# oriolfornes/ExplaiNN

Measured on AMD Instinct MI355X. Metric: sequences/sec (fwd+bwd), 200bp one-hot, 300 units, batch 1024, higher is better.
Workload: dtype f32

## Files before the change

explainn_amd/csrc/api.hip:

```cpp
#include <stdarg.h>
#include <stdio.h>
#include <string.h>

#include <cstdlib>
#include <cstring>

#include "common.h"

static thread_local char g_err[512] = "";

void explainn_set_error(const char* fmt, ...) {
    va_list ap;
    va_start(ap, fmt);
    vsnprintf(g_err, sizeof(g_err), fmt, ap);
    va_end(ap);
}

extern "C" const char* explainn_last_error(void) { return g_err; }

namespace {
struct Carver {
    int64_t off = 0;
    char* base = nullptr;
    template <typename T>
// ... 22 lines not shown
    cv.take(&c->Wsg, (int64_t)conv_tiles_padded(c->U, c->k) * 32);
    const int64_t Upad = (int64_t)32 * conv_tiles_padded(c->U, c->k);
    cv.take(&c->ext, Upad * n * Bs + 64);
    cv.take(&c->idx, Upad * n * Bs + 64);
    cv.take(&c->qs0, U * NS);
    cv.take(&c->qS1p, U * c->QCH * NS);
    cv.take(&c->qS2p, U * c->QCH * NS * NS);
    cv.take(&c->qbar, U * NS);
    cv.take(&c->VC, U * FC_H * NS);
    cv.take(&c->A2, U * FC_H * NS);
    cv.take(&c->A2f, c->NQ <= FC_BF_MAXN ? 0 : U * FC_MT * fc_nk4q(c->NQ) * 256);
    cv.take(&c->A2h, c->NQ <= FC_BF_MAXN ? U * FC_MT * fc_ks32(c->NQ) * 3 * 256 : 0);
    cv.take(&c->sh2, U * FC_H);
    cv.take(&c->sig2, U * FC_H);
    cv.take(&c->z, U * Bs);
    cv.take(&c->zhat, U * Bs);
    cv.take(&c->o, U * Bs);
    cv.take(&c->sig3, U);
    c->ZBLK = fc_fwd_blocks((int)Bs, c->NQ);
    cv.take(&c->z12p, U * c->ZBLK * 2);
    cv.take(&c->bits, U * Bs + 4);
    cv.take(&c->dz, U * Bs + 4);
    cv.take(&c->EQp, U * c->ACH * FC_H * NS);
    cv.take(&c->Sep, U * c->ACH * FC_H);
    cv.take(&c->EQs, U * FC_H * NS);
    cv.take(&c->Ttf, U * fc_nw16(c->NQ) * 3 * 4 * 256);
    cv.take(&c->Mff, U * fc_nw16(c->NQ) * 4 * fc_nw16(c->NQ) * 64);
    cv.take(&c->k0p, U * NS);
    cv.take(&c->dy, U4 * n * Bs);
    cv.take(&c->S12p, U * fc_ng(c->NQ) * (Bs / 16) * 2);
    cv.take(&c->Dspp, U * (Bs / 4) * K4);
    cv.take(&c->dlogits, (int64_t)c->maxB * c->T);
    cv.take(&c->flags, 64);
    cv.take(&c->dlT, (int64_t)c->T * Bs);
    cv.take(&c->gWp, c->T > HEAD_GEMM_MIN_T ? (int64_t)head_gw_chunks(c->maxB) * c->T * (c->U + 1) : 0);
    cv.take(&c->lossp, 256);
    cv.take(&c->site_cnt, U4 * Bs);
    cv.take(&c->site_off, U4 * Bs);
    cv.off = (cv.off + 255) & ~int64_t(255);
}

int check_batch(const explainn_ctx* c, int B) {
    if (!c) { explainn_set_error("null context"); return EXPLAINN_E_ARG; }
    if (B < 1 || B > c->maxB) {
        explainn_set_error("batch %d outside [1, max_batch=%d]", B, c->maxB);
        return EXPLAINN_E_ARG;
    }
    return EXPLAINN_OK;
}

#define TRY(call)                    \
    do {                             \
        int rc_ = (call);            \
        if (rc_ != EXPLAINN_OK) return rc_; \
    } while (0)

const char* const kStageNames[ST_COUNT] = {
    "pack_tables", "moments", "prep1_stats", "conv_pool", "qmom", "prep2", "fc_fwd", "head_fwd",
    "loss", "head_bwd", "passA", "mid", "passB", "conv_bwd", "fin_bwd"};
#define STAGE(id, call)                                                                 \
    do {                                                                                \
        if (c->timing) HIP_TRY(hipEventRecord(c->ev0[id], s));                          \
        TRY(call);                                                                      \
        if (c->timing) { HIP_TRY(hipEventRecord(c->ev1[id], s)); c->timed |= 1u << (id); } \
    } while (0)

// ... 187 lines not shown
}

extern "C" int explainn_forward_train(explainn_ctx* c, const float* x, int B,
                                      const explainn_params* p, const uint8_t* keep_mask,
                                      float dropout_p, uint64_t seed, float* logits, void* stream) {
    TRY(check_batch(c, B));
    if (B == 1) {
        explainn_set_error("Expected more than 1 value per channel when training, got input size "
                           "[1, %d, 1]", FC_H * c->U);
        return EXPLAINN_E_BATCH1;
    }
    if (dropout_p < 0.f || dropout_p >= 1.f) {
        explainn_set_error("dropout_p must be in [0,1)");
        return EXPLAINN_E_ARG;
    }
    hipStream_t s = static_cast<hipStream_t>(stream);
    c->fwd_B = 0;
    c->eval_valid = false;
    c->dense_x = nullptr;
    if (c->dense) {
        if (!x) { explainn_set_error("dense input mode needs x"); return EXPLAINN_E_ARG; }
        c->staged_B = 0;
        STAGE(ST_PACK, launch_prep1_tables(c, p, s));
        STAGE(ST_MOMENTS, launch_dense_moments(c, x, B, s));
        STAGE(ST_PREP1, launch_prep1(c, p, B, true, s));
        STAGE(ST_CONV_POOL, launch_dense_conv_pool(c, x, p, B, s));
        c->dense_x = x;
    } else {
    if (x) STAGE(ST_PACK, launch_pack_tables(c, x, p, B, s));
    else {
        TRY(launch_pack(c, x, B, false, s));
        STAGE(ST_PACK, launch_prep1_tables(c, p, s));
    }
    STAGE(ST_MOMENTS, launch_moments(c, B, s));
    STAGE(ST_PREP1, launch_prep1(c, p, B, true, s));
    STAGE(ST_CONV_POOL, launch_conv_pool(c, p, B, true, s));
    }
    STAGE(ST_QMOM, launch_qmoments(c, B, s));
    STAGE(ST_PREP2, launch_prep2(c, p, B, true, s));
    STAGE(ST_FC_FWD, launch_fc_fwd(c, p, B, true, keep_mask, dropout_p, seed, s));
    STAGE(ST_HEAD_FWD, launch_head_fwd(c, p, B, true, logits, nullptr, s));
    c->fwd_B = B;
    return EXPLAINN_OK;
}

namespace {
int backward_fc(explainn_ctx* c, int B, const explainn_params* p, const explainn_grads* g,
                const pa_head_args* head, hipStream_t s) {
    STAGE(ST_PASSA, launch_passA(c, B, head, s));
    STAGE(ST_MID, launch_mid_bwd(c, p, g, B, s));
    return EXPLAINN_OK;
}

int backward_conv(explainn_ctx* c, int B, const explainn_params* p, const explainn_grads* g,
                  int freeze_top_n_filters, hipStream_t s) {
    STAGE(ST_PASSB, launch_passB(c, B, s));
    if (c->dense_x) STAGE(ST_CONV_BWD, launch_dense_conv_bwd(c, c->dense_x, B, s));
    else STAGE(ST_CONV_BWD, launch_conv_bwd(c, B, s));
    STAGE(ST_FIN, launch_fin_bwd(c, p, g, B, freeze_top_n_filters, s));
    return EXPLAINN_OK;
}

bool head_rides_in_passA(const explainn_ctx* c, int B) { return c->T <= PA_HEAD_MAX_T && B <= 512; }

pa_head_args head_in_passA(explainn_ctx* c, const explainn_params* p, const explainn_grads* g, int mode,
                           const float* dl, int kind, const float* logits, const float* y,
                           float* loss_out) {
    pa_head_args h = {mode, c->T, kind, dl, logits, y, loss_out, p->final_w, p->bn3_w, c->o, c->zhat,
                      c->sig3, c->dz, g->final_w, g->final_b, g->bn3_w, g->bn3_b, g->fc2_b};
// ... 166 lines not shown
```

explainn_amd/csrc/common.h:

```cpp
#pragma once
#include <hip/hip_runtime.h>
#include <stdint.h>

#include "../../include/explainn_hip.h"

#define FC_H 100
#define HEAD_RB 8
#define HEAD_GEMM_MIN_T 8
#define HEAD_GW_MAXCH 32
__host__ inline int head_gw_chunks(int B) { int c = (B + 127) / 128; return c < 1 ? 1 : (c > HEAD_GW_MAXCH ? HEAD_GW_MAXCH : c); }
#define POOLW 7
#define BN_EPS_D 1e-5
#define BN_MOM_D 0.1
#define WAVE 64
#define MAX_K 32
#define MAX_NQ 160

struct explainn_ctx {
    int U, k, L, T, maxB, device;
    int Lo, n;
    int U4, Uq;
    int NQ, NS;
    int Bs;
    int K4;
// ... 33 lines not shown
    float* A2f;
    float* A2h;
    float* sh2;
    float* sig2;
    float* z;
    float* zhat;
    float* o;
    float* sig3;
    double* z12p;
    int ZBLK;
    uint4* bits;
    float* dz;
    float* EQp;
    float* Sep;
    float* EQs;
    float* Ttf;
    float* Mff;
    float* k0p;
    float* dy;
    float* S12p;
    float* Dspp;
    int dsp_stride, dsp_count;
    float* dlogits;
    float* dlT;
    int loss_blocks, loss_n; float* loss_out;
    float* gWp;
    double* lossp;
    int staged_B;
    bool eval_valid;
    uint64_t eval_version;
    bool dense;
    const float* dense_x;
    int* flags;
    int* site_cnt;
    int* site_off;
};

enum explainn_stage {
    ST_PACK, ST_MOMENTS, ST_PREP1, ST_CONV_POOL, ST_QMOM, ST_PREP2, ST_FC_FWD, ST_HEAD_FWD, ST_LOSS,
    ST_HEAD_BWD, ST_PASSA, ST_MID, ST_PASSB, ST_CONV_BWD, ST_FIN, ST_COUNT
};

void explainn_set_error(const char* fmt, ...);
#define HIP_TRY(expr)                                                              \
    do {                                                                           \
        hipError_t e_ = (expr);                                                    \
        if (e_ != hipSuccess) {                                                    \
            explainn_set_error("%s failed: %s (%s:%d)", #expr, hipGetErrorString(e_), \
                               __FILE__, __LINE__);                                \
            (void)hipGetLastError();   \
            return EXPLAINN_E_HIP;                                                 \
        }                                                                          \
    } while (0)
#define LAUNCH_CHECK()  HIP_TRY(hipGetLastError())

int launch_pack(explainn_ctx* c, const float* x, int B, bool counts, hipStream_t s);
int launch_prep1(explainn_ctx* c, const explainn_params* p, int B, bool train, hipStream_t s);
int launch_moments(explainn_ctx* c, int B, hipStream_t s);
int launch_prep1_tables(explainn_ctx* c, const explainn_params* p, hipStream_t s);
int launch_conv_pool(explainn_ctx* c, const explainn_params* p, int B, bool want_idx, hipStream_t s);
int launch_pack_tables(explainn_ctx* c, const float* x, const explainn_params* p, int B, hipStream_t s);
int launch_pack_codes(explainn_ctx* c, const uint8_t* codes, int B, int rc, hipStream_t s);
int launch_conv_act(explainn_ctx* c, int B, float* acts, hipStream_t s);
int launch_filter_act_max(explainn_ctx* c, int B, const uint8_t* select, float* umax, hipStream_t s);
int launch_filter_sites(explainn_ctx* c, int B, const uint8_t* select, const float* thr, int cap,
                        int* site_total, int* pfm, uint8_t* hit, hipStream_t s);
int launch_qmoments(explainn_ctx* c, int B, hipStream_t s);
int launch_prep2(explainn_ctx* c, const explainn_params* p, int B, bool train, hipStream_t s);
int launch_fc_fwd(explainn_ctx* c, const explainn_params* p, int B, bool train,
                  const uint8_t* keep_mask, float drop_p, uint64_t seed, hipStream_t s);
int launch_head_fwd(explainn_ctx* c, const explainn_params* p, int B, bool train, float* logits,
                    float* outs, hipStream_t s);
int launch_loss_deferred(explainn_ctx* c, int kind, const float* logits, const float* y, int B, float* loss,
                         float* dlogits, hipStream_t s);
int launch_loss(explainn_ctx* c, int kind, const float* logits, const float* y, int B,
                float* loss, float* dlogits, hipStream_t s);
int launch_head_bwd(explainn_ctx* c, const explainn_params* p, const explainn_grads* g,
                    const float* dlogits, int B, hipStream_t s);
int launch_head_bwd_fused_loss(explainn_ctx* c, const explainn_params* p, const explainn_grads* g,
                               int kind, const float* logits, const float* y, float* loss_out, int B,
                               hipStream_t s);
#define PA_HEAD_MAX_T 4
struct pa_head_args {
    int mode, T, kind;
    const float *dl, *logits, *y;
    float* loss_out;
    const float *Wf, *g3, *o, *zhat, *sig3;
    float *dz, *gWf, *gbf, *gg3, *gb3, *gc2;
};
int launch_passA(explainn_ctx* c, int B, const pa_head_args* head, hipStream_t s);
int launch_mid_bwd(explainn_ctx* c, const explainn_params* p, const explainn_grads* g, int B,
                   hipStream_t s);
int launch_passB(explainn_ctx* c, int B, hipStream_t s);
// ... 54 lines not shown
    const float sgn = (u < U && gamma1[u] < 0.f) ? -1.f : 1.f;
    if (tid == 0) Wsg[((u >> 5) * 2 + ((u >> 2) & 1)) * 16 + 4 * ((u & 31) >> 3) + (u & 3)] = sgn < 0.f ? 0x80000000u : 0u;
    for (int kk = tid; kk < 16 * KS; kk += nthreads) {
        const int j = kk >> 2, a = kk & 3;
        const float wv = j < k ? sgn * wsh[a * k + j] : 0.f;
        const uint32_t hb = __float_as_uint(wv) & 0xffff0000u;
        const float r1 = wv - __uint_as_float(hb);
        const uint32_t mb = __float_as_uint(r1) & 0xffff0000u;
        const float r2 = r1 - __uint_as_float(mb);
        const int ks = kk >> 4, lane = 32 * ((kk >> 3) & 1) + (u & 31), e = kk & 7;
        uint16_t* dst = Wf + ((((size_t)(u >> 5) * KS + ks) * 3) * 64 + lane) * 8 + e;
        dst[0] = (uint16_t)(hb >> 16);
        dst[512] = (uint16_t)(mb >> 16);
        dst[1024] = (uint16_t)(__float_as_uint(r2) >> 16);
    }
}

#ifndef EXPLAINN_XCD_MAP
#define EXPLAINN_XCD_MAP 1
#endif
__device__ __forceinline__ bool unit_chunk_of_block(int U, int& u, int& chunk) {
#if EXPLAINN_XCD_MAP
    const int G = gridDim.x, L = blockIdx.y * G + blockIdx.x;
    const int slot = L >> 3;
    u = (slot / G) * 8 + (L & 7);
    chunk = slot - (slot / G) * G;
#else
    u = blockIdx.y; chunk = blockIdx.x;
#endif
    return u < U;
}
__host__ inline int units_grid(int U) { return (U + 7) & ~7; }

__device__ __forceinline__ float qval(float alpha, float ext, float shift) {
    return __expf(fmaf(alpha, ext, shift));
}

__device__ __forceinline__ float wave_sum(float v) {
#pragma unroll
    for (int off = 32; off > 0; off >>= 1) v += __shfl_xor(v, off, 64);
    return v;
}
__device__ __forceinline__ double wave_sum_d(double v) {
#pragma unroll
    for (int off = 32; off > 0; off >>= 1) v += __shfl_xor(v, off, 64);
    return v;
}

__host__ __device__ constexpr int chunk_count(int len) { return (len + 35) / 36; }
__host__ __device__ constexpr int chunk_len(int len) {
    return (((len + chunk_count(len) - 1) / chunk_count(len)) + 3) & ~3;
}
__host__ __device__ constexpr int ns_stride(int NQ) { return chunk_count(NQ) * chunk_len(NQ); }

static inline int nq_bucket(int n) {
    static const int b[] = {4, 8, 12, 16, 20, 24, 26, 28, 32, 40, 48, 56, 64, 72, 84, 96,
                            112, 128, 140, 160};
    for (unsigned i = 0; i < sizeof(b) / sizeof(b[0]); ++i)
        if (b[i] >= n) return b[i];
    return 0;
}
__host__ __device__ constexpr int nq_lower(int NQ) {
    constexpr int b[] = {0, 4, 8, 12, 16, 20, 24, 26, 28, 32, 40, 48, 56, 64, 72, 84, 96, 112, 128, 140, 160};
    int lo = 0;
    for (int i = 1; i < 21; ++i) if (b[i] == NQ) lo = b[i - 1];
    return lo;
// ... 33 lines not shown
```

explainn_amd/csrc/convpool.hip:

```cpp
#include <cstdlib>
#include <type_traits>

#include "common.h"

typedef __attribute__((ext_vector_type(8))) __bf16 cbf16x8;
typedef float cf32x16 __attribute__((ext_vector_type(16)));
typedef uint32_t cu32x4 __attribute__((ext_vector_type(4)));

template <int KS, int UT> struct cpm_state {
    cu32x4 Wr[UT][KS][3];
    cf32x16 acc[3][UT];
    float best[UT][16];
    uint32_t arg[UT][16];
    cu32x4 bop[3][KS];
    uint32_t xs[3], nx[2];
    uint32_t gw[4], mw[3];
    uint32_t smask[UT][16];
    uint32_t so, so4;
    uint32_t r1, r5;
};
struct cpm_args {
    const uint32_t* pk2; const uint32_t* nmask; float* ext; uint8_t* idx;
    int n, Bs, PW, NW, t0, b, kh; uint32_t tbase;
    uint32_t row1, row5;
// ... 155 lines not shown
                    cpm_update_sel<KS, UT, IDX, PI, RP>(S, (e - 1) / 16, (e - 1) % 16, gt[(e - 1) % 3]);
                    cpm_update_sel<KS, UT, IDX, PI, RP>(S, e / 16, e % 16, gt[e % 3]);
                }
            } else {
                constexpr int e = k - SC::E0 - SC::NE;
                cpm_store<KS, UT, IDX>(S, A, e / 16, e % 16);
            }
        });
        __builtin_amdgcn_sched_barrier(0);
    });
}

template <int KS, int UT, bool IDX>
__device__ __forceinline__ void cpm_window(cpm_state<KS, UT>& S, const cpm_args& A, int w) {
    cpm_position<KS, UT, IDX, 0>(S, A, w);
    cpm_position<KS, UT, IDX, 1>(S, A, w);
    cpm_position<KS, UT, IDX, 2>(S, A, w);
    cpm_position<KS, UT, IDX, 3>(S, A, w);
    cpm_position<KS, UT, IDX, 4>(S, A, w);
    cpm_position<KS, UT, IDX, 5>(S, A, w);
    cpm_position<KS, UT, IDX, 6>(S, A, w);
}

template <int KS, int UT>
__device__ __forceinline__ void cpm_load_fragments(cpm_state<KS, UT>& S, const cu32x4* wsrc) {
    cpm_static_for<0, UT * KS * 3>([&S, wsrc](auto ic) {
        constexpr int i = decltype(ic)::value;
        cu32x4& dst = S.Wr[i / (KS * 3)][(i / 3) % KS][i % 3];
        const cu32x4* src = wsrc + 64 * i;
        asm volatile("global_load_dwordx4 %0, %1, off" : "=a"(dst) : "v"(src));
    });
}

template <int KS, int UT, bool IDX>
__global__ __launch_bounds__(64, (UT == 1 && KS <= 5) ? 2 : 1) void conv_pool_mm_kernel(
    const uint32_t* __restrict__ pk2, const uint32_t* __restrict__ nmask,
    const cu32x4* __restrict__ Wf, const cu32x4* __restrict__ Wsg,
    float* __restrict__ ext, uint8_t* __restrict__ idx, int n, int Bs, int PW, int NW, int wper) {
    __shared__ __attribute__((aligned(1024))) cu32x4 oh[64];
    typedef __attribute__((address_space(3))) char lds_char;
    const int lane = threadIdx.x;
    STAMP(0);
    {
        const int c4 = lane & 15, nb = lane >> 4;
        uint32_t r[4] = {0u, 0u, 0u, 0u};
#pragma unroll
        for (int h = 0; h < 2; ++h) {
            const int cde = (c4 >> (2 * h)) & 3;
            const uint32_t one = ((nb >> h) & 1) ? 0u : 0x3F80u;
#pragma unroll
            for (int q = 0; q < 4; ++q)
                if (q == 2 * h + (cde >> 1)) r[q] = one << (16 * (cde & 1));
        }
        oh[lane] = cu32x4{r[0], r[1], r[2], r[3]};
    }
    cpm_state<KS, UT> S;
    cpm_args A;
    A.pk2 = pk2; A.nmask = nmask; A.ext = ext; A.idx = idx; A.n = n; A.Bs = Bs; A.PW = PW; A.NW = NW;
    A.t0 = blockIdx.y * UT; A.b = blockIdx.x * 32 + (lane & 31); A.kh = lane >> 5;
    A.tbase = (uint32_t)(size_t)(const lds_char*)oh;
    A.row1 = (uint32_t)(n * Bs); A.row5 = 5u * A.row1;
    {
        const size_t row0 = (size_t)32 * A.t0 * n * Bs;
        const int span = __builtin_amdgcn_readfirstlane(32 * UT * n * Bs);
        auto uniform = [](auto* q) {
            const unsigned long long v = reinterpret_cast<unsigned long long>(q);
            const unsigned lo = __builtin_amdgcn_readfirstlane((unsigned)v), hi = __builtin_amdgcn_readfirstlane((unsigned)(v >> 32));
            return reinterpret_cast<decltype(q)>(((unsigned long long)hi << 32) | lo);
        };
        A.rext = __builtin_amdgcn_make_buffer_rsrc(uniform(ext + row0), 0, 4 * span, 0x00020000);
        A.ridx = __builtin_amdgcn_make_buffer_rsrc(uniform(idx + row0), 0, span, 0x00020000);
    }
    const int wbeg = blockIdx.z * wper, wend = min(n, wbeg + wper);
    if (wbeg >= wend) return;
    cpm_load_fragments(S, Wf + (size_t)A.t0 * KS * 3 * 64 + lane);
    cpm_fetch(S, A, wbeg);
    {
        const cu32x4* ssrc = Wsg + ((size_t)A.t0 * 2 + A.kh) * 4;
#pragma unroll
        for (int t = 0; t < UT; ++t)
#pragma unroll
            for (int q = 0; q < 4; ++q) {
                const cu32x4 v = ssrc[t * 8 + q];
#pragma unroll
                for (int i = 0; i < 4; ++i) S.smask[t][4 * q + i] = v[i];
            }
    }
    asm volatile("s_waitcnt vmcnt(0)" ::: "memory");
    __syncthreads();
    STAMP(1);
    cpm_window_words(S, A, wbeg);
    cpm_static_for<0, KS>([&](auto kc) { cpm_operand<KS, UT, 0, decltype(kc)::value, 0>(S, A); });
    STAMP(2);
#pragma unroll 1
    for (int w = wbeg; w < wend; ++w) {
        const bool first = w == wbeg;
        S.so = first ? CPM_OOB : cpm_store_origin(A, w - 1);
        S.so4 = first ? CPM_OOB : 4u * S.so;
        S.r1 = first ? 0u : A.row1; S.r5 = first ? 0u : A.row5;
        cpm_window<KS, UT, IDX>(S, A, w);
        if (first) STAMP(3);
    }
    STAMP(4);
    __builtin_amdgcn_sched_barrier(0);
    asm volatile("s_nop 15\n\ts_nop 15\n\ts_nop 15" ::: "memory");
    __builtin_amdgcn_sched_barrier(0);
// ... 2 lines not shown
#pragma unroll
        for (int r = 0; r < 16; ++r) cpm_update<KS, UT, IDX, POOLW - 1, 2>(S, t, r);
    S.so = cpm_store_origin(A, wend - 1);
    S.so4 = 4u * S.so;
    S.r1 = A.row1; S.r5 = A.row5;
#pragma unroll
    for (int t = 0; t < UT; ++t)
#pragma unroll
        for (int r = 0; r < 16; ++r) cpm_store<KS, UT, IDX>(S, A, t, r);
    STAMP(5);
}

static int conv_pool_mm_ut(const explainn_ctx* c) {
    if (const char* e = getenv("EXPLAINN_CPM_UT")) { const int v = atoi(e); if (v == 1 || (v == 2 && conv_ksteps(c->k) <= 5)) return v; }
    return conv_ut(c->k);
}

static int conv_pool_mm_parts(const explainn_ctx* c, int B, int ut) {
    if (const char* e = getenv("EXPLAINN_CPM_PARTS")) { const int v = atoi(e); if (v >= 1) return min(v, c->n); }
    const int groups = ut == 1 ? (c->U + 31) / 32 : conv_tiles_padded(c->U, c->k) / ut, sb = (B + 31) / 32;
    const int cols = groups * sb, slots = (ut == 1 && conv_ksteps(c->k) <= 5) ? 2048 : 1024;
    int best = 1;
    long best_cost = -1;
    for (int p = 1; p <= c->n; ++p) {
        const int wper = (c->n + p - 1) / p, np = (c->n + wper - 1) / wper;
        if (np != p) continue;
        const long rounds = ((long)cols * np + slots - 1) / slots;
        const long cost = rounds * (wper + 1);
        if (best_cost < 0 || cost < best_cost) { best_cost = cost; best = p; }
    }
    return best;
}

int launch_conv_pool_mm(explainn_ctx* c, const explainn_params* p, int B, bool want_idx, hipStream_t s) {
    const int ut = conv_pool_mm_ut(c);
    const int parts = conv_pool_mm_parts(c, B, ut);
    const int wper = (c->n + parts - 1) / parts;
    const dim3 grid((B + 31) / 32, ut == 1 ? (c->U + 31) / 32 : conv_tiles_padded(c->U, c->k) / ut, (c->n + wper - 1) / wper);
#define ARGS grid, dim3(64), 0, s, c->pk2, c->nmask, reinterpret_cast<const cu32x4*>(c->Wf), \
             reinterpret_cast<const cu32x4*>(c->Wsg), c->ext, c->idx, c->n, c->Bs, c->PW, c->NW, wper
#define CALLKS(KSv, UTv)                                                                        \
    if (want_idx) hipLaunchKernelGGL((conv_pool_mm_kernel<KSv, UTv, true>), ARGS);              \
    else hipLaunchKernelGGL((conv_pool_mm_kernel<KSv, UTv, false>), ARGS);
#define CALLUT(KSv) if (ut == 2) { CALLKS(KSv, 2); } else { CALLKS(KSv, 1); }
    switch (conv_ksteps(c->k)) {
#ifndef CPM_ONLY5
        case 1: { CALLUT(1); } break;
        case 2: { CALLUT(2); } break;
        case 3: { CALLUT(3); } break;
        case 4: { CALLUT(4); } break;
        case 6: { CALLKS(6, 1); } break;
        case 7: { CALLKS(7, 1); } break;
        case 8: { CALLKS(8, 1); } break;
#endif
        case 5: { CALLUT(5); } break;
        default: explainn_set_error("kernel_size %d not instantiated (2..32)", c->k); return EXPLAINN_E_UNSUPPORTED;
    }
#undef CALLUT
#undef CALLKS
#undef ARGS
    LAUNCH_CHECK();
    return EXPLAINN_OK;
}

int launch_conv_pool(explainn_ctx* c, const explainn_params* p, int B, bool want_idx, hipStream_t s) {
    return launch_conv_pool_mm(c, p, B, want_idx, s);
}

__global__ __launch_bounds__(256) void conv_act_kernel(const uint8_t* __restrict__ codesT,
                                                       const float* __restrict__ Wt,
                                                       const float* __restrict__ alpha,
                                                       const float* __restrict__ shift,
                                                       float* __restrict__ acts, int U, int k,
                                                       int L, int Lo, int Bs) {
    extern __shared__ float4 Wsm[];
    uint8_t* cs = reinterpret_cast<uint8_t*>(Wsm + k * 5);
    const int b = blockIdx.x, quad = blockIdx.y;
    const float4* src = reinterpret_cast<const float4*>(Wt) + (size_t)quad * k * 5;
    for (int i = threadIdx.x; i < k * 5; i += 256) Wsm[i] = src[i];
    for (int p = threadIdx.x; p < L; p += 256) cs[p] = codesT[(size_t)p * Bs + b];
    __syncthreads();
    for (int p = threadIdx.x; p < Lo; p += 256) {
        float4 acc = make_float4(0.f, 0.f, 0.f, 0.f);
        for (int j = 0; j < k; ++j) {
            const float4 v = Wsm[j * 5 + cs[p + j]];
            acc.x += v.x; acc.y += v.y; acc.z += v.z; acc.w += v.w;
        }
        const float av[4] = {acc.x, acc.y, acc.z, acc.w};
#pragma unroll
        for (int uu = 0; uu < 4; ++uu) {
            const int u = quad * 4 + uu;
            if (u < U) acts[((size_t)b * U + u) * Lo + p] = qval(alpha[u], av[uu], shift[u]);
        }
    }
}

int launch_conv_act(explainn_ctx* c, int B, float* acts, hipStream_t s) {
    const size_t sm = (size_t)c->k * 5 * sizeof(float4) + ((c->L + 15) & ~15);
    hipLaunchKernelGGL(conv_act_kernel, dim3(B, c->Uq), dim3(256), sm, s, c->codesT, c->Wt, c->alpha,
// ... 5 lines not shown
```

explainn_amd/csrc/pack.hip:

```cpp
#include "common.h"

__device__ __forceinline__ int gridDim_x_tiles(int B) { return (B + 63) / 64; }
#define PACK_WAVES 8

template <bool CODES>
__device__ __forceinline__ void pack_tile(const float* __restrict__ x,
                                          const uint8_t* __restrict__ codes_in, int rc,
                                          uint8_t* __restrict__ codesT, uint32_t* __restrict__ pk2,
                                          uint32_t* __restrict__ nmask, int B, int L, int Bs, int PW,
                                          int NW, int* __restrict__ flags, int bx, int by,
                                          unsigned long long* __restrict__ bm, int Lp) {
    __shared__ uint8_t tile[64][68];
    const int b0 = bx * 64, p0 = by * 64;
    const int lane = threadIdx.x & 63, q = threadIdx.x >> 6;
    int bad = 0;
    const int p = p0 + lane;
    const int pc = min(p, L - 1);
    if (CODES) {
        const int ps = rc ? L - 1 - pc : pc;
        for (int i0 = q; i0 < 64; i0 += 4 * PACK_WAVES) {
            int v[4];
#pragma unroll
            for (int r = 0; r < 4; ++r) v[r] = codes_in[(size_t)min(b0 + i0 + PACK_WAVES * r, B - 1) * L + ps];
#pragma unroll
// ... 73 lines not shown
            }
        }
        const int a = lane >> 4, pq = p0 + 16 * q + (lane & 15);
        if (pq < Lp) bm[((size_t)a * gridDim_x_tiles(B) + bx) * Lp + pq] = mine;
    }
    if (bad) atomicOr(flags, 1);
}

template <bool CODES>
__global__ __launch_bounds__(64 * PACK_WAVES) void pack_onehot_kernel(const float* __restrict__ x,
                                                          const uint8_t* __restrict__ codes_in,
                                                          int rc,
                                                          uint8_t* __restrict__ codesT,
                                                          uint32_t* __restrict__ pk2,
                                                          uint32_t* __restrict__ nmask, int B,
                                                          int L, int Bs, int PW, int NW,
                                                          int* __restrict__ flags,
                                                          unsigned long long* __restrict__ bm, int Lp) {
    pack_tile<CODES>(x, codes_in, rc, codesT, pk2, nmask, B, L, Bs, PW, NW, flags, blockIdx.x, blockIdx.y,
                     bm, Lp);
}

__global__ __launch_bounds__(64 * PACK_WAVES) void pack_tables_kernel(const float* __restrict__ x,
                                                          uint8_t* __restrict__ codesT,
                                                          uint32_t* __restrict__ pk2,
                                                          uint32_t* __restrict__ nmask, int B,
                                                          int L, int Bs, int PW, int NW,
                                                          int* __restrict__ flags, int gx, int gy,
                                                          const float* __restrict__ conv_w,
                                                          const float* __restrict__ gamma1,
                                                          float* __restrict__ Wt,
                                                          uint16_t* __restrict__ Wf,
                                                          uint32_t* __restrict__ Wsg, int U, int k,
                                                          unsigned long long* __restrict__ bm, int Lp) {
    __shared__ float wsh[4 * MAX_K];
    const int blk = blockIdx.x;
    if (blk < gx * gy)
        pack_tile<false>(x, nullptr, 0, codesT, pk2, nmask, B, L, Bs, PW, NW, flags, blk % gx, blk / gx,
                         bm, Lp);
    else
        filter_tables_unit(conv_w, gamma1, Wt, Wf, Wsg, U, k, blk - gx * gy, threadIdx.x, 64 * PACK_WAVES, wsh);
}

__global__ __launch_bounds__(256) void moments_kernel(const unsigned long long* __restrict__ bm,
                                                      double* __restrict__ G, double* __restrict__ m,
                                                      int B, int L, int k, int Lp) {
    extern __shared__ int cq[];
    const int d = blockIdx.x >> 4, a = (blockIdx.x >> 2) & 3, a2 = blockIdx.x & 3;
    const int tid = threadIdx.x, NT = (B + 63) / 64, Lo = L - k + 1, K4 = 4 * k;
    const unsigned long long* __restrict__ m0 = bm + (size_t)a * NT * Lp;
    const unsigned long long* __restrict__ m1 = bm + (size_t)a2 * NT * Lp + d;
    long long part = 0;
    for (int q = tid; q < L; q += 256) {
        int c = 0;
        if (q + d < L) {
            for (int t0 = 0; t0 < NT; t0 += 8) {
                unsigned long long x0[8], x1[8];
#pragma unroll
                for (int i = 0; i < 8; ++i) {
                    const size_t o = (size_t)min(t0 + i, NT - 1) * Lp + q;
                    x0[i] = m0[o]; x1[i] = m1[o];
                }
#pragma unroll
                for (int i = 0; i < 8; ++i) c += (t0 + i < NT) ? __popcll(x0[i] & x1[i]) : 0;
            }
        }
        cq[q] = c;
        if (q < Lo) part += c;
    }
// ... 8 lines not shown
        for (int q = 0; q < j; ++q) sj += cq[Lo + q] - cq[q];
        const double v = (double)sj / ((double)B * (double)Lo);
        const int row = a * k + j, col = a2 * k + j + d;
        G[(size_t)row * K4 + col] = v;
        G[(size_t)col * K4 + row] = v;
        if (row == col) m[row] = v;
    }
}

int launch_pack(explainn_ctx* c, const float* x, int B, bool counts, hipStream_t s) {
    const int gb = (B + 63) / 64;
    if (x == nullptr) {
        if (c->staged_B != B) {
            explainn_set_error("x is NULL but %s (batch %d)", c->staged_B ? "the staged codes hold "
                               "another batch size" : "no codes are staged", B);
            return EXPLAINN_E_STATE;
        }
    } else {
        c->staged_B = 0;
        hipLaunchKernelGGL(pack_onehot_kernel<false>, dim3(gb, (c->NW * 32 + 63) / 64), dim3(64 * PACK_WAVES), 0,
                           s, x, (const uint8_t*)nullptr, 0, c->codesT, c->pk2, c->nmask, B, c->L,
                           c->Bs, c->PW, c->NW, c->flags, counts ? c->bm : nullptr, c->Lp);
        LAUNCH_CHECK();
    }
    return EXPLAINN_OK;
}

int launch_pack_tables(explainn_ctx* c, const float* x, const explainn_params* p, int B,
                       hipStream_t s) {
    const int gx = (B + 63) / 64, gy = (c->NW * 32 + 63) / 64;
    c->staged_B = 0;
    hipLaunchKernelGGL(pack_tables_kernel, dim3(gx * gy + c->U4), dim3(64 * PACK_WAVES), 0, s, x, c->codesT,
                       c->pk2, c->nmask, B, c->L, c->Bs, c->PW, c->NW, c->flags, gx, gy, p->conv_w,
                       p->bn1_w, c->Wt, c->Wf, c->Wsg, c->U, c->k, c->bm, c->Lp);
    LAUNCH_CHECK();
    return EXPLAINN_OK;
}

int launch_pack_codes(explainn_ctx* c, const uint8_t* codes, int B, int rc, hipStream_t s) {
    hipLaunchKernelGGL(pack_onehot_kernel<true>, dim3((B + 63) / 64, (c->NW * 32 + 63) / 64),
                       dim3(64 * PACK_WAVES), 0, s, (const float*)nullptr, codes, rc, c->codesT, c->pk2, c->nmask,
                       B, c->L, c->Bs, c->PW, c->NW, c->flags, c->bm, c->Lp);
    LAUNCH_CHECK();
    c->staged_B = B;
    return EXPLAINN_OK;
}

int launch_moments(explainn_ctx* c, int B, hipStream_t s) {
    const size_t sm = (size_t)((c->L + 1) & ~1) * sizeof(int) + 4 * sizeof(long long);
    hipLaunchKernelGGL(moments_kernel, dim3(c->k * 16), dim3(256), sm, s, c->bm, c->G, c->m, B, c->L,
                       c->k, c->Lp);
    LAUNCH_CHECK();
    return EXPLAINN_OK;
}
```

explainn_amd/csrc/prep.hip:

```cpp
#include "common.h"

__device__ __forceinline__ double block_sum_128(double v, double* red) {
    v = wave_sum_d(v);
    const int w = threadIdx.x >> 6;
    __syncthreads();
    if ((threadIdx.x & 63) == 0) red[w] = v;
    __syncthreads();
    return red[0] + red[1];
}

__global__ __launch_bounds__(128) void prep1_tables_kernel(const float* __restrict__ conv_w,
                                                           const float* __restrict__ gamma1,
                                                           float* __restrict__ Wt,
                                                           uint16_t* __restrict__ Wf,
                                                           uint32_t* __restrict__ Wsg, int U, int k) {
    __shared__ float wsh[4 * MAX_K];
    filter_tables_unit(conv_w, gamma1, Wt, Wf, Wsg, U, k, blockIdx.x, threadIdx.x, 128, wsh);
}

template <bool TRAIN>
__global__ __launch_bounds__(128) void prep1_stats_kernel(
    const float* __restrict__ conv_w, const float* __restrict__ conv_b,
    const float* __restrict__ g1, const float* __restrict__ b1, float* __restrict__ rm,
    float* __restrict__ rv, int64_t* nbt, const double* __restrict__ G,
    const double* __restrict__ m, float* __restrict__ alpha, float* __restrict__ shift,
    double* __restrict__ mug, double* __restrict__ sig1, double* __restrict__ Gw, int U, int k,
    int B, int Lo) {
    __shared__ double wsh[4 * MAX_K];
    __shared__ double red[2];
    const int u = blockIdx.x, tid = threadIdx.x, K4 = 4 * k;
    if (u >= U) {
        if (tid == 0) { alpha[u] = 0.f; shift[u] = 0.f; }
        return;
    }
    if (!TRAIN) {
        if (tid == 0) {
            const double a = (double)g1[u] / sqrt((double)rv[u] + BN_EPS_D);
            alpha[u] = (float)a;
            shift[u] = (float)((double)b1[u] + a * ((double)conv_b[u] - (double)rm[u]));
        }
        return;
    }
    const int mi = min(tid, K4 - 1);
    const float wme = conv_w[(size_t)u * K4 + mi];
    const double mme = m[mi];
    const float g1u = g1[u], b1u = b1[u], cbu = conv_b[u], rmu = rm[u], rvu = rv[u];
    for (int i = tid + 128; i < K4; i += 128) wsh[i] = (double)conv_w[(size_t)u * K4 + i];
    extern __shared__ double Gs[];
    {
        const int n2 = K4 * K4;
        constexpr int GQ = 48;
        for (int e0 = tid; e0 < n2; e0 += 128 * GQ) {
            double gv[GQ];
#pragma unroll
            for (int q = 0; q < GQ; ++q) gv[q] = G[min(e0 + q * 128, n2 - 1)];
#pragma unroll
            for (int q = 0; q < GQ; ++q)
                if (e0 + q * 128 < n2) Gs[e0 + q * 128] = gv[q];
        }
    }
    if (tid < K4) wsh[tid] = (double)wme;
    __syncthreads();
    double mu_p = 0, q_p = 0;
    for (int i = tid; i < K4; i += 128) {
        double g0 = 0, g1s = 0;
        int c0 = 0;
        for (; c0 + 1 < K4; c0 += 2) {
            g0 = fma(Gs[c0 * K4 + i], wsh[c0], g0);
            g1s = fma(Gs[(c0 + 1) * K4 + i], wsh[c0 + 1], g1s);
        }
        if (c0 < K4) g0 = fma(Gs[c0 * K4 + i], wsh[c0], g0);
        const double gw = g0 + g1s;
        Gw[(size_t)u * K4 + i] = gw;
        mu_p = fma(wsh[i], i == tid ? mme : m[i], mu_p);
        q_p = fma(wsh[i], gw, q_p);
    }
    const double mu = block_sum_128(mu_p, red);
    const double wGw = block_sum_128(q_p, red);
    if (tid == 0) {
        double var = wGw - mu * mu;
        var = var > 0 ? var : 0;
        const double sg = sqrt(var + BN_EPS_D);
        const double a = (double)g1u / sg;
        alpha[u] = (float)a;
        shift[u] = (float)((double)b1u - a * mu);
        mug[u] = mu;
        sig1[u] = sg;
        const double N1 = (double)B * (double)Lo;
        rm[u] = (float)((1 - BN_MOM_D) * (double)rmu + BN_MOM_D * ((double)cbu + mu));
        rv[u] = (float)((1 - BN_MOM_D) * (double)rvu + BN_MOM_D * var * N1 / (N1 - 1));
        if (u == 0 && nbt) *nbt += 1;
    }
}

int launch_prep1_tables(explainn_ctx* c, const explainn_params* p, hipStream_t s) {
    hipLaunchKernelGGL(prep1_tables_kernel, dim3(c->U4), dim3(128), 0, s, p->conv_w, p->bn1_w, c->Wt,
                       c->Wf, c->Wsg, c->U, c->k);
    LAUNCH_CHECK();
    return EXPLAINN_OK;
}

int launch_prep1(explainn_ctx* c, const explainn_params* p, int B, bool train, hipStream_t s) {
    if (train)
        hipLaunchKernelGGL(prep1_stats_kernel<true>, dim3(c->U4), dim3(128),
                           (size_t)c->K4 * c->K4 * sizeof(double), s, p->conv_w,
                           p->conv_b, p->bn1_w, p->bn1_b, p->bn1_rm, p->bn1_rv, p->bn1_nbt, c->G,
                           c->m, c->alpha, c->shift, c->mug, c->sig1, c->Gw, c->U, c->k, B, c->Lo);
    else
        hipLaunchKernelGGL(prep1_stats_kernel<false>, dim3(c->U4), dim3(128), 0, s, p->conv_w,
                           p->conv_b, p->bn1_w, p->bn1_b, p->bn1_rm, p->bn1_rv, (int64_t*)nullptr,
                           c->G, c->m, c->alpha, c->shift, c->mug, c->sig1, c->Gw, c->U, c->k, B,
                           c->Lo);
    LAUNCH_CHECK();
    return EXPLAINN_OK;
}

typedef float f32x16q __attribute__((ext_vector_type(16)));
typedef float f32x4q __attribute__((ext_vector_type(4)));
#define QT_LD 65
#define QS_LD 66

template <int NQ>
__global__ __launch_bounds__(64) void qmom_kernel(
    const float* __restrict__ ext, const float* __restrict__ alpha,
    const float* __restrict__ shift, float* __restrict__ qs0, float* __restrict__ S1p,
    float* __restrict__ S2p, int n, int Bs, int B, int QCH) {
    constexpr int NS = ns_stride(NQ), NW16 = fc_nw16(NQ), ROWS = 16 * NW16;
    constexpr int NP = NW16 * (NW16 + 1) / 2;
    __shared__ float tq[ROWS * QS_LD];
    const int u = blockIdx.y, ch = blockIdx.x, lane = threadIdx.x;
// ... 529 lines not shown
```

include/explainn_hip.h:

```cpp
#ifndef EXPLAINN_HIP_H
#define EXPLAINN_HIP_H

#include <stdint.h>

#ifdef __cplusplus
extern "C" {
#endif

#define EXPLAINN_OK 0
#define EXPLAINN_E_ARG (-1)
#define EXPLAINN_E_HIP (-2)
#define EXPLAINN_E_BATCH1 (-3)
#define EXPLAINN_E_STATE (-4)
#define EXPLAINN_E_UNSUPPORTED (-5)

#define EXPLAINN_LOSS_BCE_WITH_LOGITS 0
#define EXPLAINN_LOSS_MSE 1

typedef struct explainn_ctx explainn_ctx;

typedef struct explainn_params {
    const float* conv_w;
    const float* conv_b;
    const float* bn1_w;
// ... 55 lines not shown
                           const explainn_params* p, const explainn_grads* g, int loss_kind,
                           float dropout_p, uint64_t seed, float* logits, float* loss_out,
                           void* stream);
int explainn_train_step_conv(explainn_ctx* ctx, int B, const explainn_params* p,
                             const explainn_grads* g, int freeze_top_n_filters, void* stream);

int explainn_unit_outputs(explainn_ctx* ctx, const float* x, int B, const explainn_params* p,
                          float* outs, void* stream);
int explainn_unit_activations(explainn_ctx* ctx, const float* x, int B, const explainn_params* p,
                              float* acts, void* stream);

int explainn_filter_act_max(explainn_ctx* ctx, const float* x, int B, const explainn_params* p,
                            const uint8_t* select, float* unit_max, void* stream);
int explainn_filter_sites(explainn_ctx* ctx, const float* x, int B, const explainn_params* p,
                          const uint8_t* select, const float* thresholds, int site_cap,
                          int32_t* site_total, int32_t* pfm, uint8_t* hit, void* stream);

int explainn_stage_codes(explainn_ctx* ctx, const uint8_t* codes, int B, int reverse_complement,
                         void* stream);

int explainn_stage_onehot(explainn_ctx* ctx, const float* x, int B, void* stream);

int explainn_dense_input(explainn_ctx* ctx, int enable);

#define EXPLAINN_PWM_SUM 0
#define EXPLAINN_PWM_MAX 1
int explainn_pwm_scan(const float* x, int B, int L, const float* pwms, int G, int k, int scoring,
                      float* scores, void* stream);

int explainn_adam_step(int n_tensors, float* const* params, const float* const* grads,
                       float* const* exp_avg, float* const* exp_avg_sq, const int64_t* sizes,
                       int64_t step, double lr, double beta1, double beta2, double eps, void* stream);

int explainn_input_flags(explainn_ctx* ctx, int* flags_host, void* stream);

int explainn_stage_timing(explainn_ctx* ctx, int enable);
int explainn_stage_count(void);
const char* explainn_stage_name(int i);
int explainn_stage_times(explainn_ctx* ctx, float* us, int cap);

int explainn_debug_keep_bits(explainn_ctx* ctx, int B, uint32_t* out, void* stream);

#ifdef __cplusplus
}
#endif
#endif
```

Baseline: 5.076 million.

## Fuse BN1 moments and fold into conv-pool launch via auxiliary workgroups

In the training forward pass, the separate moments and prep1 launches are replaced by extra workgroups prepended to the conv-pool grid. These compute the BN1 Gram moments from the packed bitmaps, synchronise through an atomic ticket counter with a spin-wait and timeout flag, and then fold the per-unit alpha/shift and running stats. The intent is to remove two kernel launches and their serialization. The risks are that spin-waiting assumes the aux workgroups are co-resident, and that the conv workgroups may read alpha/shift only after they are written. It is gated by a grid-size heuristic and an env override.

```diff
diff --git a/explainn_amd/csrc/api.hip b/explainn_amd/csrc/api.hip
--- a/explainn_amd/csrc/api.hip
+++ b/explainn_amd/csrc/api.hip
@@ -78,6 +78,7 @@
     cv.take(&c->Dspp, U * (Bs / 4) * K4);
     cv.take(&c->dlogits, (int64_t)c->maxB * c->T);
     cv.take(&c->flags, 64);
+    cv.take(&c->bn1_ticket, 64);
     cv.take(&c->dlT, (int64_t)c->T * Bs);
     cv.take(&c->gWp, c->T > HEAD_GEMM_MIN_T ? (int64_t)head_gw_chunks(c->maxB) * c->T * (c->U + 1) : 0);
     cv.take(&c->lossp, 256);
@@ -331,9 +332,13 @@
         TRY(launch_pack(c, x, B, false, s));
         STAGE(ST_PACK, launch_prep1_tables(c, p, s));
     }
-    STAGE(ST_MOMENTS, launch_moments(c, B, s));
-    STAGE(ST_PREP1, launch_prep1(c, p, B, true, s));
-    STAGE(ST_CONV_POOL, launch_conv_pool(c, p, B, true, s));
+    if (const int naux = conv_pool_bn1_workgroups(c, B)) {
+        STAGE(ST_CONV_POOL, launch_conv_pool_train(c, p, B, naux, s));
+    } else {
+        STAGE(ST_MOMENTS, launch_moments(c, B, s));
+        STAGE(ST_PREP1, launch_prep1(c, p, B, true, s));
+        STAGE(ST_CONV_POOL, launch_conv_pool(c, p, B, true, s));
+    }
     }
     STAGE(ST_QMOM, launch_qmoments(c, B, s));
     STAGE(ST_PREP2, launch_prep2(c, p, B, true, s));
diff --git a/explainn_amd/csrc/common.h b/explainn_amd/csrc/common.h
--- a/explainn_amd/csrc/common.h
+++ b/explainn_amd/csrc/common.h
@@ -89,6 +89,7 @@
     bool dense;
     const float* dense_x;
     int* flags;
+    int* bn1_ticket;
     int* site_cnt;
     int* site_off;
 };
@@ -116,6 +117,8 @@
 int launch_moments(explainn_ctx* c, int B, hipStream_t s);
 int launch_prep1_tables(explainn_ctx* c, const explainn_params* p, hipStream_t s);
 int launch_conv_pool(explainn_ctx* c, const explainn_params* p, int B, bool want_idx, hipStream_t s);
+int conv_pool_bn1_workgroups(const explainn_ctx* c, int B);
+int launch_conv_pool_train(explainn_ctx* c, const explainn_params* p, int B, int naux, hipStream_t s);
 int launch_pack_tables(explainn_ctx* c, const float* x, const explainn_params* p, int B, hipStream_t s);
 int launch_pack_codes(explainn_ctx* c, const uint8_t* codes, int B, int rc, hipStream_t s);
 int launch_conv_act(explainn_ctx* c, int B, float* acts, hipStream_t s);
@@ -236,6 +239,25 @@
 }
 __host__ inline int units_grid(int U) { return (U + 7) & ~7; }
 
+__device__ __forceinline__ void bn1_fold_finish(double mu, double wGw, int u, float g1u, float b1u,
+                                                float cbu, float rmu, float rvu, int B, int Lo,
+                                                float* __restrict__ alpha, float* __restrict__ shift,
+                                                double* __restrict__ mug, double* __restrict__ sig1,
+                                                float* __restrict__ rm, float* __restrict__ rv, int64_t* nbt) {
+    double var = wGw - mu * mu;
+    var = var > 0 ? var : 0;
+    const double sg = sqrt(var + BN_EPS_D);
+    const double a = (double)g1u / sg;
+    alpha[u] = (float)a;
+    shift[u] = (float)((double)b1u - a * mu);
+    mug[u] = mu;
+    sig1[u] = sg;
+    const double N1 = (double)B * (double)Lo;
+    rm[u] = (float)((1 - BN_MOM_D) * (double)rmu + BN_MOM_D * ((double)cbu + mu));
+    rv[u] = (float)((1 - BN_MOM_D) * (double)rvu + BN_MOM_D * var * N1 / (N1 - 1));
+    if (u == 0 && nbt) *nbt += 1;
+}
+
 __device__ __forceinline__ float qval(float alpha, float ext, float shift) {
     return __expf(fmaf(alpha, ext, shift));
 }
diff --git a/explainn_amd/csrc/convpool.hip b/explainn_amd/csrc/convpool.hip
--- a/explainn_amd/csrc/convpool.hip
+++ b/explainn_amd/csrc/convpool.hip
@@ -211,14 +211,199 @@
     });
 }
 
+struct cpm_bn1_args {
+    const unsigned long long* bm; double* G; double* m;
+    const float* conv_w; const float* conv_b; const float* g1; const float* b1;
+    float* rm; float* rv; int64_t* nbt;
+    float* alpha; float* shift; double* mug; double* sig1; double* Gw;
+    int* ticket; int* flags;
+    int naux, nz;
+    int U, U4, k, B, L, Lp;
+};
+typedef __attribute__((address_space(1))) unsigned long long bn1_gu64;
+typedef __attribute__((address_space(1))) int bn1_gi32;
+template <int KS, int UT> struct bn1_cfg {
+    static constexpr bool big = UT == 2 && KS >= 2;
+    static constexpr int TQ = big ? 16 : 4;
+    static constexpr int CH = big ? 40 : 12;
+};
+#define BN1_NU 2
+#define BN1_SPIN_TICKS 10000000ull
+
+__device__ __forceinline__ void bn1_store(double* p, double v) {
+    __hip_atomic_store((bn1_gu64*)p, (unsigned long long)__double_as_longlong(v), __ATOMIC_RELAXED,
+                       __HIP_MEMORY_SCOPE_AGENT);
+}
+
+template <int BN1_TQ>
+__device__ __forceinline__ void bn1_moments_job(const cpm_bn1_args& X, int job, int lane) {
+    const int d = job >> 2, a = job & 3;
+    const int NT = (X.B + 63) / 64, Lo = X.L - X.k + 1, K4 = 4 * X.k;
+    const size_t plane = (size_t)NT * X.Lp;
+    const unsigned long long* __restrict__ m0 = X.bm + (size_t)a * plane;
+    long long carry[4] = {0, 0, 0, 0}, plo[4] = {0, 0, 0, 0}, phi[4] = {0, 0, 0, 0};
+    const int jlo = lane - 1, jhi = lane + Lo - 1;
+    for (int qb = 0; qb < X.L; qb += 64) {
+        const int q = qb + lane;
+        int c[4] = {0, 0, 0, 0};
+        if (q + d < X.L) {
+            for (int t0 = 0; t0 < NT; t0 += BN1_TQ) {
+                unsigned long long x0[BN1_TQ], x1[4][BN1_TQ];
+#pragma unroll
+                for (int i = 0; i < BN1_TQ; ++i) {
+                    const size_t o = (size_t)min(t0 + i, NT - 1) * X.Lp + q;
+                    x0[i] = m0[o];
+#pragma unroll
+                    for (int a2 = 0; a2 < 4; ++a2) x1[a2][i] = X.bm[a2 * plane + d + o];
+                }
+#pragma unroll
+                for (int i = 0; i < BN1_TQ; ++i)
+#pragma unroll
+                    for (int a2 = 0; a2 < 4; ++a2) c[a2] += (t0 + i < NT) ? __popcll(x0[i] & x1[a2][i]) : 0;
+            }
+        }
+#pragma unroll
+        for (int a2 = 0; a2 < 4; ++a2) {
+            int v = c[a2];
+#pragma unroll
+            for (int off = 1; off < 64; off <<= 1) {
+                const int y = __shfl_up(v, off, 64);
+                if (lane >= off) v += y;
+            }
+            const int vlo = __shfl(v, jlo & 63, 64), vhi = __shfl(v, jhi & 63, 64);
+            if (jlo >= qb && jlo < qb + 64) plo[a2] = carry[a2] + vlo;
+            if (jhi >= qb && jhi < qb + 64) phi[a2] = carry[a2] + vhi;
+            carry[a2] += __shfl(v, 63, 64);
+        }
+    }
+    const int j = lane;
+    if (j < X.k - d) {
+#pragma unroll
+        for (int a2 = 0; a2 < 4; ++a2) {
+            const long long sj = phi[a2] - plo[a2];
+            const double v = (double)sj / ((double)X.B * (double)Lo);
+            const int row = a * X.k + j, col = a2 * X.k + j + d;
+            bn1_store(X.G + (size_t)row * K4 + col, v);
+            bn1_store(X.G + (size_t)col * K4 + row, v);
+            if (row == col) bn1_store(X.m + row, v);
+        }
+    }
+}
+
+template <int CH>
+__device__ __forceinline__ void bn1_fold_units(const cpm_bn1_args& X, const int (&us)[BN1_NU], int nu, int lane) {
+    const int K4 = 4 * X.k, Lo = X.L - X.k + 1;
+    const int i0 = lane, i1 = lane + 64;
+    const int c0i = min(i0, K4 - 1), c1i = min(i1, K4 - 1);
+    float wl[BN1_NU][2];
+#pragma unroll
+    for (int uu = 0; uu < BN1_NU; ++uu) {
+        const int u = min(us[uu], X.U - 1);
+        wl[uu][0] = X.conv_w[(size_t)u * K4 + c0i];
+        wl[uu][1] = X.conv_w[(size_t)u * K4 + c1i];
+    }
+    const double m0 = X.m[c0i], m1 = X.m[c1i];
+    double ge[BN1_NU][2], go[BN1_NU][2];
+#pragma unroll
+    for (int uu = 0; uu < BN1_NU; ++uu) ge[uu][0] = ge[uu][1] = go[uu][0] = go[uu][1] = 0;
+    for (int cb = 0; cb < K4; cb += CH) {
+        double gv[CH][2];
+#pragma unroll
+        for (int cc = 0; cc < CH; ++cc) {
+            const int c = min(cb + cc, K4 - 1);
+            gv[cc][0] = X.G[(size_t)c * K4 + c0i];
+            gv[cc][1] = X.G[(size_t)c * K4 + c1i];
+        }
+#pragma unroll
+        for (int cc = 0; cc < CH; cc += 2) {
+            const int c = cb + cc;
+            if (c < K4) {
+#pragma unroll
+                for (int uu = 0; uu < BN1_NU; ++uu) {
+                    const float we = __int_as_float(__builtin_amdgcn_readlane(
+                        __float_as_int(c < 64 ? wl[uu][0] : wl[uu][1]), c & 63));
+                    const float wo = __int_as_float(__builtin_amdgcn_readlane(
+                        __float_as_int(c + 1 < 64 ? wl[uu][0] : wl[uu][1]), (c + 1) & 63));
+#pragma unroll
+                    for (int h = 0; h < 2; ++h) {
+                        ge[uu][h] = fma(gv[cc][h], (double)we, ge[uu][h]);
+                        go[uu][h] = fma(gv[cc + 1][h], (double)wo, go[uu][h]);
+                    }
+                }
+            }
+        }
+    }
+#pragma unroll
+    for (int uu = 0; uu < BN1_NU; ++uu) {
+        if (uu >= nu) break;
+        const int u = us[uu];
+        if (u >= X.U) {
+            if (lane == 0) { X.alpha[u] = 0.f; X.shift[u] = 0.f; }
+            continue;
+        }
+        double mu_p[2] = {0, 0}, q_p[2] = {0, 0};
+#pragma unroll
+        for (int h = 0; h < 2; ++h) {
+            const int i = h ? i1 : i0;
+            const double gw = ge[uu][h] + go[uu][h];
+            if (i < K4) {
+                X.Gw[(size_t)u * K4 + i] = gw;
+                mu_p[h] = fma((double)wl[uu][h], h ? m1 : m0, mu_p[h]);
+                q_p[h] = fma((double)wl[uu][h], gw, q_p[h]);
+            }
+        }
+        const double mu = wave_sum_d(mu_p[0]) + wave_sum_d(mu_p[1]);
+        const double wGw = wave_sum_d(q_p[0]) + wave_sum_d(q_p[1]);
+        if (lane == 0)
+            bn1_fold_finish(mu, wGw, u, X.g1[u], X.b1[u], X.conv_b[u], X.rm[u], X.rv[u], X.B, Lo, X.alpha,
+                            X.shift, X.mug, X.sig1, X.rm, X.rv, X.nbt);
+    }
+}
+
+template <int KS, int UT>
+__device__ __forceinline__ void cpm_bn1(const cpm_bn1_args& X, int id, int lane) {
+    for (int job = id; job < 4 * X.k; job += X.naux) bn1_moments_job<bn1_cfg<KS, UT>::TQ>(X, job, lane);
+    asm volatile("s_waitcnt vmcnt(0)" ::: "memory");
+    if (lane == 0) __hip_atomic_fetch_add((bn1_gi32*)X.ticket, 1, __ATOMIC_RELAXED, __HIP_MEMORY_SCOPE_AGENT);
+    const unsigned long long t0 = wall_clock64();
+    while (__builtin_amdgcn_readfirstlane(
+               __hip_atomic_load((bn1_gi32*)X.ticket, __ATOMIC_RELAXED, __HIP_MEMORY_SCOPE_AGENT)) < X.naux) {
+        if (wall_clock64() - t0 > BN1_SPIN_TICKS) {
+            if (lane == 0)
+                __hip_atomic_fetch_or((bn1_gi32*)X.flags, EXPLAINN_FLAG_BN1_TIMEOUT, __ATOMIC_RELAXED,
+                                      __HIP_MEMORY_SCOPE_AGENT);
+            return;
+        }
+        __builtin_amdgcn_s_sleep(2);
+    }
+    __builtin_amdgcn_fence(__ATOMIC_ACQUIRE, "agent");
+    for (int u0 = id; u0 < X.U4; u0 += BN1_NU * X.naux) {
+        int us[BN1_NU], nu = 0;
+#pragma unroll
+        for (int uu = 0; uu < BN1_NU; ++uu) {
+            us[uu] = u0 + uu * X.naux;
+            if (us[uu] < X.U4) nu = uu + 1;
+        }
+        bn1_fold_units<bn1_cfg<KS, UT>::CH>(X, us, nu, lane);
+    }
+}
+
 template <int KS, int UT, bool IDX>
 __global__ __launch_bounds__(64, (UT == 1 && KS <= 5) ? 2 : 1) void conv_pool_mm_kernel(
     const uint32_t* __restrict__ pk2, const uint32_t* __restrict__ nmask,
     const cu32x4* __restrict__ Wf, const cu32x4* __restrict__ Wsg,
-    float* __restrict__ ext, uint8_t* __restrict__ idx, int n, int Bs, int PW, int NW, int wper) {
+    float* __restrict__ ext, uint8_t* __restrict__ idx, int n, int Bs, int PW, int NW, int wper,
+    const cpm_bn1_args bn1) {
     __shared__ __attribute__((aligned(1024))) cu32x4 oh[64];
     typedef __attribute__((address_space(3))) char lds_char;
     const int lane = threadIdx.x;
+    if constexpr (IDX) {
+        if ((int)blockIdx.z < bn1.nz) {
+            const int id = ((int)blockIdx.z * (int)gridDim.y + (int)blockIdx.y) * (int)gridDim.x + (int)blockIdx.x;
+            if (id < bn1.naux) cpm_bn1<KS, UT>(bn1, id, lane);
+            return;
+        }
+    }
     STAMP(0);
     {
         const int c4 = lane & 15, nb = lane >> 4;
@@ -250,7 +435,7 @@
         A.rext = __builtin_amdgcn_make_buffer_rsrc(uniform(ext + row0), 0, 4 * span, 0x00020000);
         A.ridx = __builtin_amdgcn_make_buffer_rsrc(uniform(idx + row0), 0, span, 0x00020000);
     }
-    const int wbeg = blockIdx.z * wper, wend = min(n, wbeg + wper);
+    const int wbeg = (IDX ? (int)blockIdx.z - bn1.nz : (int)blockIdx.z) * wper, wend = min(n, wbeg + wper);
     if (wbeg >= wend) return;
     cpm_load_fragments(S, Wf + (size_t)A.t0 * KS * 3 * 64 + lane);
     cpm_fetch(S, A, wbeg);
@@ -319,13 +504,32 @@
     return best;
 }
 
-int launch_conv_pool_mm(explainn_ctx* c, const explainn_params* p, int B, bool want_idx, hipStream_t s) {
+int conv_pool_bn1_workgroups(const explainn_ctx* c, int B) {
+    if (const char* e = getenv("EXPLAINN_BN1_AUX")) return min(max(atoi(e), 0), 256);
     const int ut = conv_pool_mm_ut(c);
     const int parts = conv_pool_mm_parts(c, B, ut);
     const int wper = (c->n + parts - 1) / parts;
-    const dim3 grid((B + 31) / 32, ut == 1 ? (c->U + 31) / 32 : conv_tiles_padded(c->U, c->k) / ut, (c->n + wper - 1) / wper);
+    const long blocks = (long)((B + 31) / 32) * (ut == 1 ? (c->U + 31) / 32 : conv_tiles_padded(c->U, c->k) / ut) *
+                        ((c->n + wper - 1) / wper);
+    const int slots = (ut == 1 && conv_ksteps(c->k) <= 5) ? 2048 : 1024;
+    return blocks >= 768 && blocks <= slots && c->L <= 256 ? 8 * c->k : 0;
+}
+
+static int launch_conv_pool_mm(explainn_ctx* c, const explainn_params* p, int B, bool want_idx,
+                               cpm_bn1_args* bn1, hipStream_t s) {
+    const int ut = conv_pool_mm_ut(c);
+    const int parts = conv_pool_mm_parts(c, B, ut);
+    const int wper = (c->n + parts - 1) / parts;
+    dim3 grid((B + 31) / 32, ut == 1 ? (c->U + 31) / 32 : conv_tiles_padded(c->U, c->k) / ut, (c->n + wper - 1) / wper);
+    cpm_bn1_args none = {};
+    if (bn1) {
+        const int slice = (int)(grid.x * grid.y);
+        bn1->nz = (bn1->naux + slice - 1) / slice;
+        grid.z += bn1->nz;
+    }
+    const cpm_bn1_args& bn1v = bn1 ? *bn1 : none;
 #define ARGS grid, dim3(64), 0, s, c->pk2, c->nmask, reinterpret_cast<const cu32x4*>(c->Wf), \
-             reinterpret_cast<const cu32x4*>(c->Wsg), c->ext, c->idx, c->n, c->Bs, c->PW, c->NW, wper
+             reinterpret_cast<const cu32x4*>(c->Wsg), c->ext, c->idx, c->n, c->Bs, c->PW, c->NW, wper, bn1v
 #define CALLKS(KSv, UTv)                                                                        \
     if (want_idx) hipLaunchKernelGGL((conv_pool_mm_kernel<KSv, UTv, true>), ARGS);              \
     else hipLaunchKernelGGL((conv_pool_mm_kernel<KSv, UTv, false>), ARGS);
@@ -351,7 +555,14 @@
 }
 
 int launch_conv_pool(explainn_ctx* c, const explainn_params* p, int B, bool want_idx, hipStream_t s) {
-    return launch_conv_pool_mm(c, p, B, want_idx, s);
+    return launch_conv_pool_mm(c, p, B, want_idx, nullptr, s);
+}
+
+int launch_conv_pool_train(explainn_ctx* c, const explainn_params* p, int B, int naux, hipStream_t s) {
+    cpm_bn1_args a = {c->bm, c->G, c->m, p->conv_w, p->conv_b, p->bn1_w, p->bn1_b, p->bn1_rm, p->bn1_rv,
+                      p->bn1_nbt, c->alpha, c->shift, c->mug, c->sig1, c->Gw, c->bn1_ticket, c->flags,
+                      naux, 0, c->U, c->U4, c->k, B, c->L, c->Lp};
+    return launch_conv_pool_mm(c, p, B, true, &a, s);
 }
 
 __global__ __launch_bounds__(256) void conv_act_kernel(const uint8_t* __restrict__ codesT,
diff --git a/explainn_amd/csrc/pack.hip b/explainn_amd/csrc/pack.hip
--- a/explainn_amd/csrc/pack.hip
+++ b/explainn_amd/csrc/pack.hip
@@ -129,9 +129,11 @@
                                                           float* __restrict__ Wt,
                                                           uint16_t* __restrict__ Wf,
                                                           uint32_t* __restrict__ Wsg, int U, int k,
-                                                          unsigned long long* __restrict__ bm, int Lp) {
+                                                          unsigned long long* __restrict__ bm, int Lp,
+                                                          int* __restrict__ bn1_ticket) {
     __shared__ float wsh[4 * MAX_K];
     const int blk = blockIdx.x;
+    if (blk == 0 && threadIdx.x == 0) *bn1_ticket = 0;
     if (blk < gx * gy)
         pack_tile<false>(x, nullptr, 0, codesT, pk2, nmask, B, L, Bs, PW, NW, flags, blk % gx, blk / gx,
                          bm, Lp);
@@ -206,7 +208,7 @@
     c->staged_B = 0;
     hipLaunchKernelGGL(pack_tables_kernel, dim3(gx * gy + c->U4), dim3(64 * PACK_WAVES), 0, s, x, c->codesT,
                        c->pk2, c->nmask, B, c->L, c->Bs, c->PW, c->NW, c->flags, gx, gy, p->conv_w,
-                       p->bn1_w, c->Wt, c->Wf, c->Wsg, c->U, c->k, c->bm, c->Lp);
+                       p->bn1_w, c->Wt, c->Wf, c->Wsg, c->U, c->k, c->bm, c->Lp, c->bn1_ticket);
     LAUNCH_CHECK();
     return EXPLAINN_OK;
 }
diff --git a/explainn_amd/csrc/prep.hip b/explainn_amd/csrc/prep.hip
--- a/explainn_amd/csrc/prep.hip
+++ b/explainn_amd/csrc/prep.hip
@@ -13,8 +13,10 @@
                                                            const float* __restrict__ gamma1,
                                                            float* __restrict__ Wt,
                                                            uint16_t* __restrict__ Wf,
-                                                           uint32_t* __restrict__ Wsg, int U, int k) {
+                                                           uint32_t* __restrict__ Wsg, int U, int k,
+                                                           int* __restrict__ bn1_ticket) {
     __shared__ float wsh[4 * MAX_K];
+    if (blockIdx.x == 0 && threadIdx.x == 0) *bn1_ticket = 0;
     filter_tables_unit(conv_w, gamma1, Wt, Wf, Wsg, U, k, blockIdx.x, threadIdx.x, 128, wsh);
 }
 
@@ -77,25 +79,12 @@
     }
     const double mu = block_sum_128(mu_p, red);
     const double wGw = block_sum_128(q_p, red);
-    if (tid == 0) {
-        double var = wGw - mu * mu;
-        var = var > 0 ? var : 0;
-        const double sg = sqrt(var + BN_EPS_D);
-        const double a = (double)g1u / sg;
-        alpha[u] = (float)a;
-        shift[u] = (float)((double)b1u - a * mu);
-        mug[u] = mu;
-        sig1[u] = sg;
-        const double N1 = (double)B * (double)Lo;
-        rm[u] = (float)((1 - BN_MOM_D) * (double)rmu + BN_MOM_D * ((double)cbu + mu));
-        rv[u] = (float)((1 - BN_MOM_D) * (double)rvu + BN_MOM_D * var * N1 / (N1 - 1));
-        if (u == 0 && nbt) *nbt += 1;
-    }
+    if (tid == 0) bn1_fold_finish(mu, wGw, u, g1u, b1u, cbu, rmu, rvu, B, Lo, alpha, shift, mug, sig1, rm, rv, nbt);
 }
 
 int launch_prep1_tables(explainn_ctx* c, const explainn_params* p, hipStream_t s) {
     hipLaunchKernelGGL(prep1_tables_kernel, dim3(c->U4), dim3(128), 0, s, p->conv_w, p->bn1_w, c->Wt,
-                       c->Wf, c->Wsg, c->U, c->k);
+                       c->Wf, c->Wsg, c->U, c->k, c->bn1_ticket);
     LAUNCH_CHECK();
     return EXPLAINN_OK;
 }
diff --git a/include/explainn_hip.h b/include/explainn_hip.h
--- a/include/explainn_hip.h
+++ b/include/explainn_hip.h
@@ -111,6 +111,7 @@
                        float* const* exp_avg, float* const* exp_avg_sq, const int64_t* sizes,
                        int64_t step, double lr, double beta1, double beta2, double eps, void* stream);
 
+#define EXPLAINN_FLAG_BN1_TIMEOUT 2
 int explainn_input_flags(explainn_ctx* ctx, int* flags_host, void* stream);
 
 int explainn_stage_timing(explainn_ctx* ctx, int enable);
```

After: 5.229 million (median of 6 runs). +3.0%, better.
